# lefarov/Ape-X-DQN

Hardware: AMD Instinct MI355X
Metric: learner grad-steps/sec at batch 512, 84x84x4 dueling DQN (higher is better)
Workload: dtype fp32; 1 GPU; model=dueling NatureCNN (reference DuellingDQN, conv1=64), 4x84x84, A=4, global_batch=512, seq_len=1, parallelism=dp1, batch_scope=global, per_rank_rows=512, replay_per_gpu=100000, learner=fused/hip, hip_graphs=True

## Files before the change

### apex_dqn_amd/csrc/conv12_fused.hip

```cpp
#include "mfma_common.h"
#include "conv2_wfrag.h"
#include "cf_pack.h"

#define CF_THREADS 256
#define CF_PLANE 52224
#define CF_MAXIMG 64
#define CF_FRAME 7056
#define CF_NY2 12
#define CF_WAHEAD 3
#define CF_W3AHEAD 5
#define CF_W3EARLY 0

typedef float f32x16 __attribute__((ext_vector_type(16)));

struct Conv12Desc {
  const uint8_t* ring;
  const int32_t* slots;
  const float* w1;
  const float* w1b;
  const float* b1;
  const float* b1b;
  const bf16_t* w2;
  const bf16_t* w2_lo;
  const bf16_t* w2b;
// ... 3 lines not shown
  const float* b2;
  const float* b2b;
  bf16_t* y1;
  bf16_t* y1_lo;
  bf16_t* y2;
  bf16_t* y2_lo;
  uint4* w1frag;
  uint8_t* scratch;
  int N, C, img_switch, copy_n;
  float in_scale;
  uint64_t* probe;
  unsigned long long* wq;
  int bf16;
  int probe_split;
  const bf16_t* w3;
  const bf16_t* w3_lo;
  const bf16_t* w3b;
  const bf16_t* w3b_lo;
  const float* b3;
  const float* b3b;
  bf16_t* y3;
  bf16_t* y3_lo;
  uint4* w3frag;
};

template <int C>
__global__ void __launch_bounds__(256) cf_pack_kernel(CfPack p) {
  if ((int)blockIdx.x < p.nc2f) {
    c2f_pack_range(p.c2f, blockIdx.x * 256 + threadIdx.x, p.nc2f * 256);
    return;
  }
  if ((int)blockIdx.x < p.nc2f + p.nc3f) {
    c3f_pack_range(p.c3f, (blockIdx.x - p.nc2f) * 256 + threadIdx.x, p.nc3f * 256);
    return;
  }
  cf_pack_w1_block(p, C, (int)blockIdx.x - p.nc2f - p.nc3f, threadIdx.x);
}

__device__ __forceinline__ int cf_pix(int ih, int iw) { return ((ih & 1) * 2 + (iw & 1)) * 100 + (ih >> 1) * 10 + (iw >> 1); }
__device__ __forceinline__ int cf_off(int P, int c) { return (P << 7) + ((c ^ ((P >> 1) & 7)) << 4); }

__host__ __device__ constexpr int cf_young_stores(int ndw, bool split) {
  int n = 0;
  for (int q = ndw - 1; q < 12; ++q) n += (split || (q & 1) == 0) ? 1 : 0;
  return n;
}
// ... 85 lines not shown
      const float s0 = __shfl(ws, 4 * g, 64), s1 = __shfl(ws, 4 * g + 1, 64);
      const float s2 = __shfl(ws, 4 * g + 2, 64), s3 = __shfl(ws, 4 * g + 3, 64);
      bias1[nt] = (f32x4){bb.x - 1024.f * s0, bb.y - 1024.f * s1, bb.z - 1024.f * s2, bb.w - 1024.f * s3};
    }
    wf = d.wfrag + set * 2 * C2F_FRAGS + wv * 32 * 64 + lane;
    const float* B2 = set ? d.b2b : d.b2;
#pragma unroll
    for (int jh = 0; jh < 2; ++jh)
      bias2[jh] = *reinterpret_cast<const float4*>(B2 + nh * 32 + 8 * (2 * kp + jh) + 4 * kg);
    asm volatile("s_waitcnt vmcnt(0)" ::: "memory");
  };

  int q0[3];
#pragma unroll
  for (int mt = 0; mt < 3; ++mt) {
    const int r = mt * 32 + rr, oh = r / 10, ow = r - oh * 10;
    q0[mt] = (oh + kp) * 10 + ow;
  }

  const bool two = d.w1b != nullptr;
  int cur_set = -1;
  uint4 pend[3][2];
  int pend_img = -1;
  int yoff[3];
#pragma unroll
  for (int mt = 0; mt < 3; ++mt) {
    const int r = mt * 32 + rr, oh = r / 10, ow = r - oh * 10;
    yoff[mt] = (oh < 9 && ow < 9) ? ((oh * 9 + ow) * 64 + nh * 32 + 4 * kg) * 2 : -1;
  }
  auto store_y2 = [&](int q) {
    const int mt = q >> 2, jh = (q >> 1) & 1, plane = q & 1;
    const int jq = 2 * kp + jh;
    if (!SPLIT && plane) return;
    const uint8_t* base = reinterpret_cast<const uint8_t*>((plane ? d.y2_lo : d.y2) + (int64_t)pend_img * 5184);
    if (yoff[mt] >= 0) {
      const uint4 v = pend[mt][jh];
      *reinterpret_cast<uint2*>(const_cast<uint8_t*>(base) + (uint32_t)(yoff[mt] + 16 * jq)) =
          plane ? make_uint2(v.z, v.w) : make_uint2(v.x, v.y);
    }
  };
  bf16x8 wh3[CF_W3AHEAD + 1], wl3[CF_W3AHEAD + 1];
  auto w3row = [&](const int set3, const bool lo) -> const uint4* {
    return d.w3frag + (2 * set3 + (lo ? 1 : 0)) * C3F_FRAGS + (wv & 1) * 36 * 64 + lane;
  };
  auto wofs3 = [](int s) { return s * 64; };
  auto conv3_prefetch = [&](const int set3) {
// ... 108 lines not shown
            split_pk_bf16(v2, v3, h23, l23);
          } else {
            h01 = cvt_pk_bf16(v0, v1);
            h23 = cvt_pk_bf16(v2, v3);
          }
          if (oh < 7 && ow < 7) {
            const uint32_t off = (uint32_t)(((oh * 7 + ow) * 64 + c0) * 2);
            *reinterpret_cast<uint2*>(y3h + off) = make_uint2(h01, h23);
            if (SPLIT) *reinterpret_cast<uint2*>(y3l + off) = make_uint2(l01, l23);
          }
        }
      }
    }
    __syncthreads();
    if (it == 0) PROBE(d.probe, 4, PROBE_ITERS - 3, 3);
  };

  PROBE(d.probe, 4, PROBE_ITERS - 2, 0);
  if (cur < d.N) issue_dma(cur, 0);
  PROBE(d.probe, 4, PROBE_ITERS - 2, 1);
  for (int i = 0; cur < d.N; ++i) {
    const int img = cur;
    const bool more = nxt < d.N;
    const int set = (two && img >= d.img_switch) ? 1 : 0;
    if (set != cur_set) {
#ifdef APEX_PROBE
      if (i == 0 && (d.probe_split & 1)) asm volatile("s_waitcnt vmcnt(0)" ::: "memory");
      if (i == 0) PROBE(d.probe, 4, PROBE_ITERS - 2, 2);
#endif
      load_weights(set);
      cur_set = set;
      if (i == 0) PROBE(d.probe, 4, PROBE_ITERS - 2, 3);
      __syncthreads();
    }
    sl4_t nsl = (sl4_t){0, 0, 0, 0};
    if (more) nsl = image_slots(nxt);
    if (tid == 0) reinterpret_cast<volatile int*>(&q_img)[0] = more ? wq_next(d.wq, wq_seq, d.N) : d.N;
    PROBE(d.probe, 4, i, 0);
    const uint8_t* S = STG + (i & 1) * STGB;
    {
      auto load_tile = [&](int j, uint2* u) {
        int p = 16 * (th + 2 * j) + pl;
        if (j == 12) p = min(p, 399);
        const int oh = p / 20, ow = p - 20 * oh;
        const uint8_t* A = S + ((oh * 21 + ow) << 4);
#pragma unroll
// ... 43 lines not shown
          }
          if (pj >= 0) {
#pragma unroll
            for (int k = s2 * 8 / (2 * C); k < (s2 + 1) * 8 / (2 * C); ++k) epi_piece(k, pj, pacc, paccl);
          }
#pragma unroll
          for (int q = 0; q < (SPLIT ? 4 : 2); ++q) {
            __builtin_amdgcn_sched_group_barrier(0x008, 1, 0);
            __builtin_amdgcn_sched_group_barrier(0x002, SPLIT ? 3 : 5, 0);
          }
          __builtin_amdgcn_sched_barrier(0);
        }
      };
      uint2 u[2][2 * C];
      f32x4 a[2][2], al[2][2];
      load_tile(0, u[0]);
      load_tile(1, u[1]);
      __builtin_amdgcn_sched_barrier(0);
      mfma_tile(u[0], a[0], al[0], -1, nullptr, nullptr);
#pragma unroll
      for (int j = 1; j < 13; ++j) {
        if (j + 1 < 13) load_tile(j + 1, u[(j + 1) & 1]);
        if (j - 1 < NDW && more) issue_dma_piece(nsl, (i + 1) & 1, j - 1);
        if (i > 0) store_y2(j - 1);
        __builtin_amdgcn_sched_barrier(0);
        mfma_tile(u[j & 1], a[j & 1], al[j & 1], j - 1, a[(j - 1) & 1], al[(j - 1) & 1]);
      }
#pragma unroll
      for (int k = 0; k < 8; ++k) epi_piece(k, 12, a[0], al[0]);
    }
    PROBE(d.probe, 4, i, 1);
    static_assert(NDW <= 7, "the vmcnt below assumes the last DMA piece at tile <= 7");
    if (i > 0) asm volatile("s_waitcnt vmcnt(%0)" ::"n"(cf_young_stores(NDW, SPLIT)) : "memory");
    else asm volatile("s_waitcnt vmcnt(0)" ::: "memory");
    __syncthreads();
    const bool copy = img < d.copy_n;
    if (copy) {
      int tq = tid;
      asm volatile("" : "+v"(tq));
      const int cst = tq & 7;
      auto store_chunk = [&](const int r, const uint4 v) {
        const int k = tq + CF_THREADS * r;
        const int plane = k >= 3200 ? 1 : 0, kk = k - plane * 3200;
        const int P = kk >> 3, c = cst ^ ((P >> 1) & 7);
        const int cls = P / 100, q = P - cls * 100, a = q / 10, b = q - a * 10;
        const int ih = 2 * a + (cls >> 1), iw = 2 * b + (cls & 1);
        *reinterpret_cast<uint4*>((plane ? d.y1_lo : d.y1) + (int64_t)img * 25600 + (ih * 20 + iw) * 64 + c * 8) = v;
      };
      constexpr int NR = SPLIT ? 25 : 12, NB = SPLIT ? 5 : 4;
#pragma unroll
      for (int r0 = 0; r0 < NR; r0 += NB) {
        uint4 v[NB];
#pragma unroll
        for (int r = 0; r < NB; ++r)
          v[r] = *reinterpret_cast<const uint4*>(
              Y1 + (r0 + r) * 4096 + tq * 16 +
// ... 78 lines not shown
          const float v1 = fmaxf((bb.y + p0.y) + p1.y, 0.f);
          const float v2 = fmaxf((bb.z + p0.z) + p1.z, 0.f);
          const float v3 = fmaxf((bb.w + p0.w) + p1.w, 0.f);
          uint32_t h01, l01 = 0, h23, l23 = 0;
          if (SPLIT) {
            split_pk_bf16(v0, v1, h01, l01);
            split_pk_bf16(v2, v3, h23, l23);
          } else {
            h01 = cvt_pk_bf16(v0, v1);
            h23 = cvt_pk_bf16(v2, v3);
          }
          pend[mt][jh] = make_uint4(h01, h23, l01, l23);
        }
      }
    };
    if (kp == 0) finish(0, true);
    else finish(2, false);
    pend_img = img;
    __syncthreads();
    if (d.w3 != nullptr) conv3_image(img, set, STG + (i & 1) * STGB, i);
    cur = nxt;
    nxt = nn;
  }
  if (pend_img >= 0) {
#pragma unroll
    for (int q = 0; q < 12; ++q) store_y2(q);
  }
  PROBE(d.probe, 4, PROBE_ITERS - 1, 1);
#ifdef APEX_PROBE
  asm volatile("s_waitcnt vmcnt(0)" ::: "memory");
  if (d.probe != nullptr && blockIdx.x < PROBE_BLOCKS && (threadIdx.x & 63) == 0)
    d.probe[((blockIdx.x * 4 + (threadIdx.x >> 6)) * PROBE_ITERS + PROBE_ITERS - 1) * 4 + 3] =
        __builtin_amdgcn_s_memrealtime();
#endif
}

static int cf_launch_pack(const Conv12Desc& d, hipStream_t st) {
  const int sets = d.pack_sets & ((d.w1b != nullptr) ? 3 : 1);
  if (sets == 0) return 0;
  const bool s0 = sets & 1, s1 = (sets & 2) != 0;
  const bool c3 = d.w3 != nullptr && d.w3frag != nullptr;
  CfPack pk{C2fPack{{s0 ? d.w2 : nullptr, s0 ? d.w2_lo : nullptr, s1 ? d.w2b : nullptr, s1 ? d.w2b_lo : nullptr},
                    d.wfrag, 0},
            (s1 ? 4 : 2) * C2F_FRAGS / 256,
            C3fPack{{c3 && s0 ? d.w3 : nullptr, c3 && s0 ? d.w3_lo : nullptr, c3 && s1 ? d.w3b : nullptr,
                     c3 && s1 ? d.w3b_lo : nullptr}, d.w3frag},
            c3 ? (s1 ? 4 : 2) * C3F_FRAGS / 256 : 0,
// ... 20 lines not shown
APEX_EXPORT int apex_conv12_fused_fwd(Conv12Desc d, int grid, hipStream_t st) {
  if (d.N < 1) return 0;
  const bool sp = d.bf16 == 0;
  if (d.ring == nullptr || d.slots == nullptr || d.w1 == nullptr || d.b1 == nullptr || d.w2 == nullptr ||
      (sp && d.w2_lo == nullptr) || d.b2 == nullptr || d.y2 == nullptr || (sp && d.y2_lo == nullptr) ||
      d.wfrag == nullptr || d.scratch == nullptr || d.w1frag == nullptr)
    return (int)hipErrorInvalidValue;
  const bool two = d.w1b != nullptr;
  if (two && (d.b1b == nullptr || d.w2b == nullptr || (sp && d.w2b_lo == nullptr) || d.b2b == nullptr))
    return (int)hipErrorInvalidValue;
  if (d.copy_n > 0 && (d.y1 == nullptr || (sp && d.y1_lo == nullptr) || d.copy_n > d.N))
    return (int)hipErrorInvalidValue;
  if (d.w3 != nullptr &&
      (d.b3 == nullptr || d.y3 == nullptr || d.w3frag == nullptr || ((uintptr_t)d.w3frag & 15) || (sp && (d.w3_lo == nullptr || d.y3_lo == nullptr)) ||
       (two && (d.w3b == nullptr || d.b3b == nullptr || (sp && d.w3b_lo == nullptr))) ||
       (((uintptr_t)d.w3 | (uintptr_t)(sp ? d.w3_lo : d.w3) | (uintptr_t)(two ? d.w3b : d.w3) |
         (uintptr_t)(two && sp ? d.w3b_lo : d.w3) | (uintptr_t)d.b3 | (uintptr_t)(two ? d.b3b : d.b3)) & 15) ||
       (((uintptr_t)d.y3 | (uintptr_t)(sp ? d.y3_lo : d.y3)) & 7)))
    return (int)hipErrorInvalidValue;
  if ((((uintptr_t)d.w1 | (uintptr_t)(two ? d.w1b : d.w1) | (uintptr_t)d.b1 | (uintptr_t)(two ? d.b1b : d.b1) |
        (uintptr_t)d.w2 | (uintptr_t)d.w2_lo | (uintptr_t)d.b2 | (uintptr_t)d.y1 | (uintptr_t)d.y1_lo) & 15) ||
      (((uintptr_t)d.y2 | (uintptr_t)d.y2_lo | (uintptr_t)d.scratch) & 7) || ((uintptr_t)d.wfrag & 15))
    return (int)hipErrorInvalidValue;
  int G = grid > 0 ? grid : 256;
  if (G > d.N) G = d.N;
  if ((d.N + G - 1) / G > CF_MAXIMG) G = (d.N + CF_MAXIMG - 1) / CF_MAXIMG;
  const int err = cf_launch_pack(d, st);
  if (err) return err;
  switch (d.C * 2 + (sp ? 1 : 0)) {
    case 3: conv12_fused_kernel<1, true><<<G, CF_THREADS, 0, st>>>(d); break;
    case 5: conv12_fused_kernel<2, true><<<G, CF_THREADS, 0, st>>>(d); break;
    case 9: conv12_fused_kernel<4, true><<<G, CF_THREADS, 0, st>>>(d); break;
    case 2: conv12_fused_kernel<1, false><<<G, CF_THREADS, 0, st>>>(d); break;
    case 4: conv12_fused_kernel<2, false><<<G, CF_THREADS, 0, st>>>(d); break;
    case 8: conv12_fused_kernel<4, false><<<G, CF_THREADS, 0, st>>>(d); break;
    default: return (int)hipErrorInvalidValue;
  }
  APEX_CHECK_LAUNCH();
}
```

### apex_dqn_amd/learner/fused_learner.py

```python
from __future__ import annotations

from typing import Any, Dict, Optional

import torch

from ..config import ApexConfig
from ..models.dueling import DuellingDQN
from ..models.flat_params import (FlatLayout, flat_to_reference_state, nature_segments,
                                  reference_state_to_flat)
from ..ops.fused_ops import HipBackend, TorchBackend, split_into
from ..ops.switches import SW
from ..utils.checkpoint import (adopt_obs_scale, check_dist_head, check_noisy, layout_segments, load_checkpoint,
                                pack_flat_state, save_checkpoint, unpack_flat_state, checkpoint_network)
from .dp_step import DataParallelStep, Streams
from .is_norm import IsNormMixin
from .schedules import StepIndexMixin, target_ema_on


def _enable_sharding(replay, comm, rt, mcap: int = 0) -> None:
    if not replay.sharded:
        seed0 = comm.broadcast_int(int(rt.seed)) if hasattr(comm, "broadcast_int") else int(rt.seed)
        replay.enable_sharding(comm.rank, comm.world_size, shard_seed=(seed0 << 20) ^ 0x5EED,
                               group=comm.group, mcap=mcap)
    replay.shard_mcap = int(mcap)
# ... 303 lines not shown
        return kw if self.split else {}

    @property
    def _conv123(self) -> bool:
        return bool(self._c12) and 0 < 3 * self.B <= SW.conv123_max_images

    @property
    def _rows_first(self) -> int:
        return self.B if self.munchausen else 2 * self.B

    def forward_all(self, defer_head: bool = False) -> None:
        ops, rt, B = self.ops, self.rt, self.B
        Pb, P, Tb, T, Pl, Tl = self.Pb, self.P, self.Tb, self.T, self.Pl, self.Tl
        sp = self.split
        n, r1 = 3 * B, self._rows_first
        ring, slots = self._frame_src()
        if self._c12:
            c1, c2 = self._conv12_weights()
            online = 0 if self._frag_out is not None else 1
            c3 = self._conv3_weights() if self._conv123 else None
            ops.conv12_fwd(ring, slots, self.frames, rt.obs_scale, self.y1, self.y1_lo, self.y2,
                           self.y2_lo, c1, c2, rows_first=r1, copy_n=B,
                           pack_sets=online | (0 if self._tgt_current() else 2), c3=c3, y3=self.y3,
                           y3_lo=self.y3_lo)
        else:
            c2f = (Pb["w2"], None, Tb["w2"], None)
            ops.conv1_fwd_ring(ring, slots, self.frames, Pb["w1"], P["b1"], rt.obs_scale, self.y1,
                               Tb["w1"], T["b1"], r1, c2f=c2f)
            ops.conv_fwd(self.y1, Pb["w2"], P["b2"], 2, self.y2, Tb["w2"], T["b2"], r1)
        self._issue_params()
        if not self._conv123:
            ops.conv_fwd(self.y2, Pb["w3"], P["b3"], 1, self.y3, Tb["w3"], T["b3"], r1,
                         **self._lo(x_lo=self.y2_lo, w_lo=sp and Pl["w3"], w2_lo=sp and Tl["w3"], out_lo=self.y3_lo))
        self._wait_params()
        wfc, wfc_lo, bfc, wfc_t, wfc_t_lo, bfc_t = self._fc_weights()
        ops.fc_fwd(self.y3.reshape(n, 3136), wfc, bfc, self.h, wfc_t, bfc_t, r1,
                   c2d=(Pb["w2"], Pl["w2"] if sp else None), defer_head=defer_head,
                   **self._lo(x_lo=sp and self.y3_lo.reshape(n, 3136), w_lo=wfc_lo,
                              w2_lo=wfc_t_lo, out_lo=self.h_lo))

    def _conv12_weights(self):
        P, T, Pb, Tb, Pl, Tl = self.P, self.T, self.Pb, self.Tb, self.Pl, self.Tl
        sp = self.split
        return ((P["w1"], P["b1"], T["w1"], T["b1"]),
                (Pb["w2"], Pl["w2"] if sp else None, P["b2"], Tb["w2"], Tl["w2"] if sp else None, T["b2"]))

    def _conv3_weights(self):
# ... 606 lines not shown
```

### apex_dqn_amd/ops/conv.py

```python
from __future__ import annotations

from typing import Dict, Optional, Tuple


import torch

from . import _lib
from .switches import SW


class Workspace:
    def __init__(self):
        self.bufs: Dict[Tuple, torch.Tensor] = {}

    def get(self, key, numel: int, device, dtype=torch.float32) -> torch.Tensor:
        k = (key, numel, str(device), dtype)
        t = self.bufs.get(k)
        if t is None:
            t = torch.empty(numel, dtype=dtype, device=device)
            self.bufs[k] = t
        return t

    work_queue = False

# ... 201 lines not shown


def conv12_frag_out(ws: "Workspace", w1: torch.Tensor, w1_off: int, w2_off: int, scale: float,
                    w3_off: Optional[int] = None, target: bool = False):
    C = int(w1.shape[1])
    dev = w1.device
    fo = _lib.CfFragOut()
    s = 1 if target else 0
    fo.w1frag = ws.get(("cf_w1frag",), CF_W1FRAG_BYTES, dev, torch.uint8).data_ptr() + s * 1024 * C * 16
    fo.c2f = ws.get(("cf_c2f_wfrag",), 4 * 8192 * 16, dev, torch.uint8).data_ptr() + s * 2 * 8192 * 16
    fo.w1_off, fo.w2_off, fo.C, fo.in_scale = int(w1_off), int(w2_off), C, float(scale)
    if w3_off is not None:
        fo.c3f = ws.get(("cf_c3f",), C3F_BYTES, dev, torch.uint8).data_ptr() + s * 2 * 4608 * 16
        fo.w3_off = int(w3_off)
    return fo


def conv12_fused_fwd(lib, ws: "Workspace", ring: torch.Tensor, slots: torch.Tensor, w1: torch.Tensor,
                     b1: torch.Tensor, w2: torch.Tensor, w2_lo: torch.Tensor, b2: torch.Tensor, scale: float,
                     y2: torch.Tensor, y2_lo: torch.Tensor, y1: Optional[torch.Tensor] = None,
                     y1_lo: Optional[torch.Tensor] = None, copy_n: int = 0, w1b=None, b1b=None, w2b=None,
                     w2b_lo=None, b2b=None, rows_first: int = 0, grid: int = 0,
                     probe: Optional[torch.Tensor] = None, pack_sets: int = 3, probe_split: int = 0,
                     c3=None, y3: Optional[torch.Tensor] = None, y3_lo: Optional[torch.Tensor] = None) -> None:
    N, C = slots.shape
    sp = w2_lo is not None
    assert slots.dtype == torch.int32 and slots.is_contiguous() and int(w1.shape[1]) == C
    assert tuple(y2.shape[:4]) == (N, 9, 9, 64) and y2.is_contiguous() and y2.dtype == torch.bfloat16
    assert not sp or (y2_lo is not None and tuple(y2_lo.shape) == (N, 9, 9, 64))
    d = _conv12_desc(ws, ring, slots, w1, b1, w2, w2_lo, b2, scale, w1b, b1b, w2b, w2b_lo, b2b, c3)
    d.img_switch = int(rows_first) if w1b is not None else N
    if copy_n > 0:
        assert y1 is not None and (y1_lo is not None or not sp) and y1.shape[0] >= copy_n and \
            tuple(y1.shape[1:]) == (20, 20, 64) and y1.is_contiguous()
        d.y1, d.y1_lo = y1.data_ptr(), (y1_lo.data_ptr() if sp else 0)
    d.copy_n = int(copy_n)
    d.y2, d.y2_lo = y2.data_ptr(), (y2_lo.data_ptr() if sp else 0)
    d.pack_sets = int(pack_sets)
    d.N = N
    d.probe = _lib.ptr(probe)
    d.probe_split = int(probe_split)
    d.wq = ws.wq(("cf_wq", N, int(grid)), ring.device, overlapped=False)
    if c3 is not None:
        assert y3 is not None and tuple(y3.shape[:4]) == (N, 7, 7, 64) and y3.is_contiguous()
        assert not sp or (y3_lo is not None and tuple(y3_lo.shape[:4]) == (N, 7, 7, 64))
        d.y3, d.y3_lo = y3.data_ptr(), (y3_lo.data_ptr() if sp else 0)
    _lib.check(lib.apex_conv12_fused_fwd(d, int(grid), _lib.stream_ptr()), "conv12_fused_fwd")


def conv_fwd(lib, x: torch.Tensor, w: torch.Tensor, b: torch.Tensor, stride: int, out: torch.Tensor,
             w2=None, b2=None, rows_first: int = 0, x_lo=None, w_lo=None, w2_lo=None, out_lo=None,
             packed: bool = False) -> None:
    N, H, W, Cin = x.shape
    Cout, KH, KW, _ = w.shape
    OH, OW = out.shape[1], out.shape[2]
    if SW.conv2_img and (H, W, Cin, Cout, KH, KW, stride) == (20, 20, 64, 64, 4, 4, 2) and \
            hasattr(lib, "apex_conv2_img_fwd"):
        conv2_img_fwd(lib, x, w, b, out, w2, b2, rows_first, x_lo=x_lo, w_lo=w_lo, w2_lo=w2_lo, out_lo=out_lo,
                      packed=packed)
        return
    d = _conv_desc(x=x.data_ptr(), w=w.data_ptr(), bias=b.data_ptr(), y=out.data_ptr(), N=N, H=H, W=W,
                   Cin=Cin, OH=OH, OW=OW, Cout=Cout, KH=KH, KW=KW, stride=stride, mode=1, relu=1,
# ... 172 lines not shown

def _splits(Mred: int, target_rows: int, max_rows: int) -> Tuple[int, int]:
    rows = max(_WG_ROWS, min(max_rows, (target_rows // _WG_ROWS) * _WG_ROWS))
    return (Mred + rows - 1) // rows, rows


def conv2_wgrad_rows_covers(x_shape, dy_shape, KH: int, stride: int, split: bool, rows: int) -> bool:
    return (bool(split) and KH == 4 and stride == 2 and len(x_shape) == 4 and len(dy_shape) == 4
            and tuple(x_shape[1:]) == (20, 20, 64) and tuple(dy_shape[1:]) == (9, 9, 64)
            and x_shape[0] == dy_shape[0] and x_shape[0] > 0
            and rows > 0 and rows % _WG_ROWS == 0 and rows <= _WG_TBL)


def conv2_wgrad_rows_pick(x_shape, dy_shape, KH: int, stride: int, split: bool, rows: int,
                          force: Optional[bool] = None) -> bool:
    covers = conv2_wgrad_rows_covers(x_shape, dy_shape, KH, stride, split, rows)
    if force is not None:
        if force and not covers:
            raise ValueError("conv2_wgrad_rows does not cover this problem")
        return bool(force)
    return covers and bool(SW.conv2_wgrad_rows) and x_shape[0] >= SW.conv2_wgrad_rows_min


def conv_wgrad(lib, ws: Workspace, dy: torch.Tensor, x: torch.Tensor, KH: int, stride: int,
               dw_out: torch.Tensor, db_out: torch.Tensor, target_rows: int = 0, jobs: Optional[list] = None,
               dy_lo=None, x_lo=None, rows_kernel: Optional[bool] = None) -> None:
    N, OH, OW, Co = dy.shape
    if target_rows <= 0:
        small = N < 256
        target_rows = {3: SW.wg_rows3, 4: SW.wg_rows2}.get(KH) or \
            ((192 if small else 384) if KH == 3 else (352 if small else 704))
    _, H, W, Cin = x.shape
    Kc = KH * KH * Cin
    Mred = N * OH * OW
    nsplit, rows = _splits(Mred, target_rows, _WG_TBL)
    slab = ws.get(("wg", Co, Kc), nsplit * Co * Kc, dy.device)
    bslab = ws.get(("wgb", Co, Kc), nsplit * Co, dy.device)
    d = _wg_desc(dy=dy.data_ptr(), x=x.data_ptr(), slab=slab.data_ptr(), bias_slab=bslab.data_ptr(), N=N,
                 H=H, W=W, Cin=Cin, OH=OH, OW=OW, KH=KH, KW=KH, stride=stride, mode=1, Co=Co, Kc=Kc, ldd=Co,
                 rows_per_split=rows, Mred=Mred, dy_lo=_lib.ptr(dy_lo), x_lo=_lib.ptr(x_lo))
    launch, what = lib.apex_conv_wgrad, "conv_wgrad"
    if conv2_wgrad_rows_pick(x.shape, dy.shape, KH, stride, dy_lo is not None and x_lo is not None, rows,
                             rows_kernel):
        launch, what = lib.apex_conv2_wgrad_rows, "conv2_wgrad_rows"
    if jobs is not None:
        _lib.check(launch(d, None, None, nsplit, 1.0, _lib.stream_ptr()), what)
        jobs.append(dict(slab=slab, bslab=bslab, out=dw_out, bout=db_out, n=Co * Kc, nsplit=nsplit, nb=Co,
                         s2dC=0, Kc=Kc, scale=1.0))
        return
    _lib.check(launch(d, dw_out.data_ptr(), db_out.data_ptr(), nsplit, 1.0, _lib.stream_ptr()), what)
# ... 208 lines not shown
```

### apex_dqn_amd/ops/conv_sigs.py

```python
from __future__ import annotations

import ctypes

c_p = ctypes.c_void_p
c_i = ctypes.c_int
c_i64 = ctypes.c_int64
c_f = ctypes.c_float


class Conv2ImgDesc(ctypes.Structure):
    _fields_ = [("x", c_p), ("w", c_p), ("w2", c_p), ("bias", c_p), ("bias2", c_p), ("y", c_p),
                ("N", c_i), ("img_switch", c_i), ("x_lo", c_p), ("w_lo", c_p), ("w2_lo", c_p), ("y_lo", c_p),
                ("wfrag", c_p), ("wfrag_ready", c_i)]


class Conv12Desc(ctypes.Structure):
    _fields_ = [("ring", c_p), ("slots", c_p), ("w1", c_p), ("w1b", c_p), ("b1", c_p), ("b1b", c_p),
                ("w2", c_p), ("w2_lo", c_p), ("w2b", c_p), ("w2b_lo", c_p), ("wfrag", c_p), ("pack_sets", c_i),
                ("b2", c_p), ("b2b", c_p), ("y1", c_p), ("y1_lo", c_p), ("y2", c_p), ("y2_lo", c_p),
                ("w1frag", c_p), ("scratch", c_p), ("N", c_i), ("C", c_i), ("img_switch", c_i), ("copy_n", c_i),
                ("in_scale", ctypes.c_float), ("probe", c_p), ("wq", c_p), ("bf16", c_i), ("probe_split", c_i),
                ("w3", c_p), ("w3_lo", c_p), ("w3b", c_p), ("w3b_lo", c_p), ("b3", c_p), ("b3b", c_p),
                ("y3", c_p), ("y3_lo", c_p), ("w3frag", c_p)]


class Conv2DgradImgDesc(ctypes.Structure):
    _fields_ = [("dy", c_p), ("w", c_p), ("mask", c_p), ("dx", c_p), ("N", c_i), ("dy_lo", c_p), ("w_lo", c_p),
                ("dx_lo", c_p), ("wfrag", c_p), ("wfrag_ready", c_i), ("wq", c_p), ("cls_split", c_i)]


class Conv21BwdDesc(ctypes.Structure):
    _fields_ = [("dy", c_p), ("dy_lo", c_p), ("w", c_p), ("w_lo", c_p), ("mask", c_p), ("wfrag", c_p),
                ("wfrag_ready", c_i), ("ring", c_p), ("slots", c_p), ("zero16", c_p), ("slab", c_p),
                ("bias_slab", c_p), ("dx", c_p), ("dx_lo", c_p), ("wq", c_p), ("N", c_i), ("C", c_i)]


class C2dPackJob(ctypes.Structure):
    _fields_ = [("w", c_p), ("w_lo", c_p), ("out", c_p)]


class Conv3DgradImgDesc(ctypes.Structure):
    _fields_ = [("dy", c_p), ("w", c_p), ("mask", c_p), ("dx", c_p), ("N", c_i)]


class Conv3DgradSplitDesc(ctypes.Structure):
    _fields_ = [("dy", c_p), ("dy_lo", c_p), ("w", c_p), ("w_lo", c_p), ("mask", c_p), ("dx", c_p),
                ("dx_lo", c_p), ("N", c_i), ("H", c_i), ("W", c_i), ("Cout", c_i), ("Cin", c_i), ("KH", c_i),
                ("KW", c_i), ("stride", c_i)]


def declare(lib: ctypes.CDLL) -> None:
    from ._lib import ConvDesc, WgradDesc
    sigs = {
        "apex_conv2_img_fwd": ([Conv2ImgDesc, c_i, c_p], c_i),
        "apex_conv12_fused_fwd": ([Conv12Desc, c_i, c_p], c_i),
        "apex_conv12_pack": ([Conv12Desc, c_p], c_i),
        "apex_conv2_dgrad_img": ([Conv2DgradImgDesc, c_i, c_p], c_i),
        "apex_conv3_dgrad_img": ([Conv3DgradImgDesc, c_i, c_p], c_i),
        "apex_conv3_dgrad_img_split": ([Conv3DgradSplitDesc, c_i, c_p], c_i),
        "apex_conv21_bwd_fused": ([Conv21BwdDesc, c_i, c_p], c_i),
        "apex_conv_fwd": ([ConvDesc, c_p], c_i),
        "apex_fc_gemm128": ([ConvDesc, c_p, c_i64, c_i, c_i, c_i, C2dPackJob, c_p], c_i),
        "apex_conv_wgrad": ([WgradDesc, c_p, c_p, c_i, c_f, c_p], c_i),
        "apex_conv2_wgrad_rows": ([WgradDesc, c_p, c_p, c_i, c_f, c_p], c_i),
        "apex_pack_dgrad_weights": ([c_p, c_p, c_p, c_p, c_p, c_p, c_p], c_i),
    }
    for name, (args, res) in sigs.items():
        fn = getattr(lib, name, None)
        if fn is None:
            continue
        fn.argtypes = args
        fn.restype = res
```

### apex_dqn_amd/ops/fused_ops.py

```python
from __future__ import annotations

import ctypes
from typing import Dict, Optional

import numpy as np
import torch

from . import _lib
from . import conv as C
from . import reference as R
from ..learner.rescale import rescale_target
from .switches import SW


def join(hi: torch.Tensor, lo: Optional[torch.Tensor], dtype=torch.float32) -> torch.Tensor:
    return hi.to(dtype) if lo is None else hi.to(dtype) + lo.to(dtype)


def _head_dtype(t: torch.Tensor):
    return torch.float64 if t.dtype == torch.float64 else torch.float32


def split_into(v: torch.Tensor, hi: torch.Tensor, lo: Optional[torch.Tensor]) -> None:
    hi.copy_(v.reshape(hi.shape))
# ... 19 lines not shown
        dt = torch.float32 if out_lo is not None else self.dtype
        split_into(R.conv1_fwd(frames, w, b, scale, dt), out, out_lo)

    def conv1_fwd_ring(self, ring, slots, frames_buf, w, b, scale, out, w2=None, b2=None, rows_first=0, w32=None,
                       w2_32=None, out_lo=None, c2f=None):
        from ..replay.gpu_replay import from_s2d
        frames = frames_buf[:slots.shape[0]]
        n, c = slots.shape
        frames.copy_(from_s2d(ring[slots.long()].reshape(n * c, 84, 84)).reshape(n, c, 84, 84))
        wa, wb = (w32, w2_32) if out_lo is not None else (w, w2)
        if w2 is None:
            self.conv1_fwd(frames, wa, b, scale, out, out_lo)
        else:
            r = rows_first
            self.conv1_fwd(frames[:r], wa, b, scale, out[:r], None if out_lo is None else out_lo[:r])
            self.conv1_fwd(frames[r:], wb, b2, scale, out[r:], None if out_lo is None else out_lo[r:])

    def conv12_pack(self, c1, c2, scale, sets=2, c3=None):
        """Repack the fused conv12 kernel's weight fragments of ``sets`` (bit 0 online, bit
        1 target; HIP backend only) -- after the target weights change; ``c3``: the fused
        conv3's too."""

    def conv12_fwd(self, ring, slots, frames_buf, scale, y1, y1_lo, y2, y2_lo, c1, c2, rows_first=0, copy_n=None,
                   pack_sets=3, c3=None, y3=None, y3_lo=None):
        w1, b1, w1b, b1b = c1
        w2, w2l, b2, w2b, w2bl, b2b = c2
        self.conv1_fwd_ring(ring, slots, frames_buf, w1.to(y1.dtype), b1, scale, y1,
                            None if w1b is None else w1b.to(y1.dtype), b1b, rows_first, w32=w1, w2_32=w1b,
                            out_lo=y1_lo)
        self.conv_fwd(y1, w2, b2, 2, y2, w2b, b2b, rows_first, x_lo=y1_lo, w_lo=w2l, w2_lo=w2bl, out_lo=y2_lo)
        if c3 is not None:
            w3, w3l, b3, w3b, w3bl, b3b = c3
            self.conv_fwd(y2, w3, b3, 1, y3, w3b, b3b, rows_first, x_lo=y2_lo, w_lo=w3l, w2_lo=w3bl, out_lo=y3_lo)

    def conv_fwd(self, x, w, b, stride, out, w2=None, b2=None, rows_first=0, x_lo=None, w_lo=None, w2_lo=None,
                 out_lo=None):
        dt = torch.float32 if x_lo is not None else self.dtype
        xf = join(x, x_lo) if x_lo is not None else x
        if w2 is None:
            split_into(R.conv_fwd(xf, join(w, w_lo), b, stride, dt), out, out_lo)
        else:
            r = rows_first
            split_into(R.conv_fwd(xf[:r], join(w, w_lo), b, stride, dt), out[:r], None if out_lo is None else out_lo[:r])
            split_into(R.conv_fwd(xf[r:], join(w2, w2_lo), b2, stride, dt), out[r:],
                       None if out_lo is None else out_lo[r:])

    def fc_fwd(self, x, w, b, out, w2=None, b2=None, rows_first=0, x_lo=None, w_lo=None, w2_lo=None, out_lo=None,
# ... 612 lines not shown
    def conv1_fwd_ring(self, ring, slots, frames_buf, w, b, scale, out, w2=None, b2=None, rows_first=0, w32=None,
                       w2_32=None, out_lo=None, c2f=None):
        if not self.native_conv:
            return super().conv1_fwd_ring(ring, slots, frames_buf, w, b, scale, out, w2, b2, rows_first, w32, w2_32,
                                          out_lo)
        c2f = c2f if (c2f is not None and SW.c2f_pack) else None
        C.conv1_s2d_fwd(self.lib, self.ws, ring, slots, w, b, scale, out, w2, b2, rows_first, w32=w32, w2_32=w2_32,
                        out_lo=out_lo, c2f=c2f)
        if c2f is not None:
            self._c2f_packed = tuple(_lib.ptr(t) for t in c2f)

    def _conv12_native(self) -> bool:
        return self.native_conv and SW.conv12_fused and hasattr(self.lib, "apex_conv12_fused_fwd")

    def conv12_pack(self, c1, c2, scale, sets=2, c3=None):
        if not self._conv12_native():
            return
        w1, b1, w1b, b1b = c1
        w2, w2l, b2, w2b, w2bl, b2b = c2
        C.conv12_pack(self.lib, self.ws, w1, b1, w2, w2l, b2, scale, w1b=w1b, b1b=b1b, w2b=w2b, w2b_lo=w2bl,
                      b2b=b2b, sets=sets, c3=c3)

    def conv12_fwd(self, ring, slots, frames_buf, scale, y1, y1_lo, y2, y2_lo, c1, c2, rows_first=0, copy_n=None,
                   pack_sets=3, c3=None, y3=None, y3_lo=None):
        if not self._conv12_native():
            return super().conv12_fwd(ring, slots, frames_buf, scale, y1, y1_lo, y2, y2_lo, c1, c2, rows_first,
                                      copy_n, c3=c3, y3=y3, y3_lo=y3_lo)
        w1, b1, w1b, b1b = c1
        w2, w2l, b2, w2b, w2bl, b2b = c2
        n = slots.shape[0] if copy_n is None else int(copy_n)
        C.conv12_fused_fwd(self.lib, self.ws, ring, slots, w1, b1, w2, w2l, b2, scale, y2, y2_lo, y1=y1, y1_lo=y1_lo,
                           copy_n=n, w1b=w1b, b1b=b1b, w2b=w2b, w2b_lo=w2bl, b2b=b2b, rows_first=rows_first,
                           pack_sets=pack_sets, c3=c3, y3=y3, y3_lo=y3_lo)

    def conv_fwd(self, x, w, b, stride, out, w2=None, b2=None, rows_first=0, x_lo=None, w_lo=None, w2_lo=None,
                 out_lo=None):
        if not self.native_conv:
            return super().conv_fwd(x, w, b, stride, out, w2, b2, rows_first, x_lo, w_lo, w2_lo, out_lo)
        key = (_lib.ptr(w), _lib.ptr(w_lo), _lib.ptr(w2), _lib.ptr(w2_lo))
        packed = stride == 2 and getattr(self, "_c2f_packed", None) == key
        if packed:
            self._c2f_packed = None
        C.conv_fwd(self.lib, x, w, b, stride, out, w2, b2, rows_first, x_lo=x_lo, w_lo=w_lo, w2_lo=w2_lo,
                   out_lo=out_lo, packed=packed)

    def fc_fwd(self, x, w, b, out, w2=None, b2=None, rows_first=0, x_lo=None, w_lo=None, w2_lo=None, out_lo=None,
               c2d=None, defer_head=False, ksplit=0):
        if not self.native_conv:
            return super().fc_fwd(x, w, b, out, w2, b2, rows_first, x_lo, w_lo, w2_lo, out_lo)
        M, K = x.shape[0], x[0].numel()
        if w.shape[0] % 128 == 0 and K % 64 == 0 and hasattr(self.lib, "apex_fc_gemm128"):
            defer = defer_head and w2 is not None and b is not None and b2 is not None and \
                2 * (M // 3) == rows_first and M % 3 == 0
            tiles = C.row_tiles_host(M, rows_first if w2 is not None else None, 128) * (w.shape[0] // 128)
            if ksplit > 0:
                ks = int(ksplit)
# ... 491 lines not shown
```

### apex_dqn_amd/ops/switches.py

```python
from __future__ import annotations

import dataclasses
import os
from dataclasses import dataclass
from typing import Any, Dict


@dataclass
class Switches:
    conv2_img: bool = True
    c2f_pack: bool = True
    conv12_fused: bool = True
    conv123_max_images: int = 1 << 20
    conv12_bf16: bool = True
    conv3_dgrad_img: bool = True
    conv2_dgrad_img: bool = True
    conv3_dgrad_img_split: bool = True
    conv3_dgrad_img_split_min: int = 74
    conv2_dgrad_cls_max: int = 256
    conv21_bwd_fused: bool = True
    opt_frags: bool = True
    fc_epi_in_head: bool = True
    bwd_branches: bool = True
    actor_fc_ksplit: int = 4
    fc_wgrad_main: str = "auto"
    fc_ksplit_max: int = 0
    work_queue: str = "auto"
    wg_rows3: int = 0
    wg_rows2: int = 0
    conv2_wgrad_rows: bool = True
    conv2_wgrad_rows_min: int = 512
    impala_wg_target: int = 512
    impala_slab_cap: int = 8 << 20
    resblock_r16: int = 14
    impala_pool_wgrad: bool = True
    isplit_bands: str = ""
    dp_fc_shard_branch: bool = False
    dp_branch_one_wait: bool = True
    dp_fc_split_rows: int = -1
    dp_norm_split: bool = True

    @classmethod
    def from_env(cls, spec: str = None) -> "Switches":
        sw = cls()
        spec = os.environ.get("APEX_SWITCHES", "") if spec is None else spec
        for item in spec.split(","):
            item = item.strip()
            if not item:
                continue
            if "=" not in item:
                raise ValueError(f"APEX_SWITCHES item must be name=value, got {item!r}")
            k, v = item.split("=", 1)
            f = {f.name: f for f in dataclasses.fields(cls)}.get(k)
            if f is None:
# ... 21 lines not shown
```

Baseline: 2946 grad-steps/s (batch 512).

## Skip y2 stores for target-net images and add per-image conv3 wgrad kernel

The fused conv1/2/3 forward kernel now writes y2 only for the first y2_n images (the online batch) when conv3 is fused. Target-network images never need y2 for backward, so this removes their global stores and the vmcnt wait on them. Separately, it adds a per-image double-buffered split-bf16 MFMA conv3 weight-gradient kernel with slab reduction. That kernel is gated behind a switch that defaults to off.

```diff
diff --git a/apex_dqn_amd/csrc/conv12_fused.hip b/apex_dqn_amd/csrc/conv12_fused.hip
--- a/apex_dqn_amd/csrc/conv12_fused.hip
+++ b/apex_dqn_amd/csrc/conv12_fused.hip
@@ -49,6 +49,7 @@
   bf16_t* y3;
   bf16_t* y3_lo;
   uint4* w3frag;
+  int y2_n;
 };
 
 template <int C>
@@ -180,6 +181,7 @@
   int cur_set = -1;
   uint4 pend[3][2];
   int pend_img = -1;
+  const int y2_lim = d.y2_n;
   int yoff[3];
 #pragma unroll
   for (int mt = 0; mt < 3; ++mt) {
@@ -334,6 +336,7 @@
   for (int i = 0; cur < d.N; ++i) {
     const int img = cur;
     const bool more = nxt < d.N;
+    const bool st_prev = pend_img >= 0 && pend_img < y2_lim;
     const int set = (two && img >= d.img_switch) ? 1 : 0;
     if (set != cur_set) {
 #ifdef APEX_PROBE
@@ -423,7 +426,7 @@
       for (int j = 1; j < 13; ++j) {
         if (j + 1 < 13) load_tile(j + 1, u[(j + 1) & 1]);
         if (j - 1 < NDW && more) issue_dma_piece(nsl, (i + 1) & 1, j - 1);
-        if (i > 0) store_y2(j - 1);
+        if (st_prev) store_y2(j - 1);
         __builtin_amdgcn_sched_barrier(0);
         mfma_tile(u[j & 1], a[j & 1], al[j & 1], j - 1, a[(j - 1) & 1], al[(j - 1) & 1]);
       }
@@ -432,7 +435,7 @@
     }
     PROBE(d.probe, 4, i, 1);
     static_assert(NDW <= 7, "the vmcnt below assumes the last DMA piece at tile <= 7");
-    if (i > 0) asm volatile("s_waitcnt vmcnt(%0)" ::"n"(cf_young_stores(NDW, SPLIT)) : "memory");
+    if (st_prev) asm volatile("s_waitcnt vmcnt(%0)" ::"n"(cf_young_stores(NDW, SPLIT)) : "memory");
     else asm volatile("s_waitcnt vmcnt(0)" ::: "memory");
     __syncthreads();
     const bool copy = img < d.copy_n;
@@ -557,7 +560,7 @@
     cur = nxt;
     nxt = nn;
   }
-  if (pend_img >= 0) {
+  if (pend_img >= 0 && pend_img < y2_lim) {
 #pragma unroll
     for (int q = 0; q < 12; ++q) store_y2(q);
   }
@@ -624,6 +627,7 @@
         (uintptr_t)d.w2 | (uintptr_t)d.w2_lo | (uintptr_t)d.b2 | (uintptr_t)d.y1 | (uintptr_t)d.y1_lo) & 15) ||
       (((uintptr_t)d.y2 | (uintptr_t)d.y2_lo | (uintptr_t)d.scratch) & 7) || ((uintptr_t)d.wfrag & 15))
     return (int)hipErrorInvalidValue;
+  if (d.w3 == nullptr || d.y2_n <= 0 || d.y2_n > d.N) d.y2_n = d.N;
   int G = grid > 0 ? grid : 256;
   if (G > d.N) G = d.N;
   if ((d.N + G - 1) / G > CF_MAXIMG) G = (d.N + CF_MAXIMG - 1) / CF_MAXIMG;
diff --git a/apex_dqn_amd/csrc/conv3_wgrad_img.hip b/apex_dqn_amd/csrc/conv3_wgrad_img.hip
--- /dev/null
+++ b/apex_dqn_amd/csrc/conv3_wgrad_img.hip
@@ -0,0 +1,162 @@
+#include "igemm_wgrad.h"
+
+#define C3W_THREADS 512
+#define C3W_DY 8192
+#define C3W_XROWS 88
+#define C3W_X (C3W_XROWS * 128)
+#define C3W_BUF (2 * C3W_DY + 2 * C3W_X)
+#define C3W_NPIECE (2 * 8 + 2 * 11)
+#define C3W_PPW ((C3W_NPIECE + 7) / 8)
+static_assert(2 * C3W_BUF <= 160 * 1024, "LDS");
+
+__device__ __forceinline__ bf16x8 c3w_frag(const uint8_t* img, int row0, int col0, int lane) {
+  const int g = lane >> 4, q = (lane >> 2) & 3, pcol = lane & 3;
+  const int rA = row0 + 8 * g + q;
+  const int cbyte = (col0 + 4 * pcol) * 2;
+  const int c16 = cbyte >> 4, within = cbyte & 15;
+  const lds_s16x4* pa = (const lds_s16x4*)(img + swz_tr(rA, c16) + within);
+  const lds_s16x4* pb = (const lds_s16x4*)(img + swz_tr(rA + 4, c16) + within);
+  s16x4 lo = __builtin_amdgcn_ds_read_tr16_b64_v4i16(const_cast<lds_s16x4*>(pa));
+  s16x4 hi = __builtin_amdgcn_ds_read_tr16_b64_v4i16(const_cast<lds_s16x4*>(pb));
+  typedef short s16x8 __attribute__((ext_vector_type(8)));
+  s16x8 v = (s16x8){lo[0], lo[1], lo[2], lo[3], hi[0], hi[1], hi[2], hi[3]};
+  return __builtin_bit_cast(bf16x8, v);
+}
+
+__global__ void __launch_bounds__(C3W_THREADS, 1) conv3_wgrad_img_kernel(WgradDesc d) {
+  __shared__ __attribute__((aligned(16))) uint8_t smem[2 * C3W_BUF];
+  const int tid = threadIdx.x, lane = tid & 63;
+  const int wv = __builtin_amdgcn_readfirstlane(tid >> 6);
+  const int ch = wv & 1, kq = wv >> 1;
+  const int b = (int)blockIdx.x, G = (int)gridDim.x;
+  const int i0 = (int)(((int64_t)b * d.N) / G), i1 = (int)(((int64_t)(b + 1) * d.N) / G);
+
+  for (int i = tid; i < 2 * C3W_BUF / 16; i += C3W_THREADS)
+    *reinterpret_cast<uint4*>(smem + i * 16) = make_uint4(0, 0, 0, 0);
+
+  uint32_t voff[C3W_PPW];
+#pragma unroll
+  for (int k = 0; k < C3W_PPW; ++k) {
+    const int p = wv + 8 * k;
+    const bool isx = p >= 16;
+    const int lp = isx ? (p - 16) % 11 : (p & 7);
+    const int R = lp * 8 + (lane >> 3);
+    const int s = ((R >> 1) & 1) | (((R >> 3) & 1) << 1);
+    const int c = (lane & 7) ^ (s << 1);
+    const int oh = R / 9, ow = R - 9 * oh;
+    const bool ok = isx ? R < 81 : (oh < 7 && ow < 7);
+    const int pix = isx ? R : oh * 7 + ow;
+    voff[k] = ok && p < C3W_NPIECE ? (uint32_t)(pix * 128 + c * 16) : 0xffffffffu;
+  }
+  const uint32_t lds0 = (uint32_t)(uintptr_t)(__attribute__((address_space(3))) uint8_t*)smem;
+  auto issue_dma = [&](int img, int buf) {
+#pragma unroll
+    for (int k = 0; k < C3W_PPW; ++k) {
+      const int p = wv + 8 * k;
+      if (p < C3W_NPIECE) {
+        const bool isx = p >= 16;
+        const bool lo = isx ? p >= 27 : p >= 8;
+        const int lp = isx ? (p - 16) % 11 : (p & 7);
+        const uint8_t* src = isx ? reinterpret_cast<const uint8_t*>(lo ? d.x_lo : d.x) + (int64_t)img * (81 * 128)
+                                 : reinterpret_cast<const uint8_t*>(lo ? d.dy_lo : d.dy) + (int64_t)img * (49 * 128);
+        const uint32_t dst = __builtin_amdgcn_readfirstlane(
+            lds0 + (uint32_t)(buf * C3W_BUF + (isx ? 2 * C3W_DY + (lo ? C3W_X : 0) : (lo ? C3W_DY : 0)) + lp * 1024));
+        if (voff[k] != 0xffffffffu) dma16_s(src, voff[k], dst);
+      }
+    }
+  };
+
+  f32x4 acc[2][9], accb[2], accb_sum[2];
+#pragma unroll
+  for (int i = 0; i < 2; ++i) {
+    accb[i] = (f32x4){0.f, 0.f, 0.f, 0.f};
+    accb_sum[i] = (f32x4){0.f, 0.f, 0.f, 0.f};
+#pragma unroll
+    for (int j = 0; j < 9; ++j) acc[i][j] = (f32x4){0.f, 0.f, 0.f, 0.f};
+  }
+  const bf16x8 ones = __builtin_bit_cast(bf16x8, make_uint4(0x3f803f80u, 0x3f803f80u, 0x3f803f80u, 0x3f803f80u));
+  const bool do_bias = d.bias_slab != nullptr && kq == 0;
+
+  __syncthreads();
+  if (i0 < i1) issue_dma(i0, 0);
+  for (int img = i0, buf = 0; img < i1; ++img, buf ^= 1) {
+    asm volatile("s_waitcnt vmcnt(0)" ::: "memory");
+    __syncthreads();
+    if (img + 1 < i1) issue_dma(img + 1, buf ^ 1);
+    const uint8_t* DH = smem + buf * C3W_BUF;
+    const uint8_t* DL = DH + C3W_DY;
+    const uint8_t* XH = DH + 2 * C3W_DY;
+    const uint8_t* XL = XH + C3W_X;
+#pragma unroll
+    for (int kk = 0; kk < 2; ++kk) {
+      bf16x8 a[2], al[2];
+#pragma unroll
+      for (int i = 0; i < 2; ++i) {
+        a[i] = c3w_frag(DH, 32 * kk, 32 * ch + 16 * i, lane);
+        al[i] = c3w_frag(DL, 32 * kk, 32 * ch + 16 * i, lane);
+      }
+#pragma unroll
+      for (int j = 0; j < 9; ++j) {
+        const int col0 = 144 * kq + 16 * j, tap = col0 >> 6, ci0 = col0 & 63;
+        const int kh = tap / 3, toff = 9 * kh + (tap - 3 * kh);
+        const bf16x8 x = c3w_frag(XH, 32 * kk + toff, ci0, lane);
+        const bf16x8 xl = c3w_frag(XL, 32 * kk + toff, ci0, lane);
+#pragma unroll
+        for (int i = 0; i < 2; ++i) {
+          acc[i][j] = __builtin_amdgcn_mfma_f32_16x16x32_bf16(x, al[i], acc[i][j], 0, 0, 0);
+          acc[i][j] = __builtin_amdgcn_mfma_f32_16x16x32_bf16(xl, a[i], acc[i][j], 0, 0, 0);
+          acc[i][j] = __builtin_amdgcn_mfma_f32_16x16x32_bf16(x, a[i], acc[i][j], 0, 0, 0);
+        }
+      }
+      if (do_bias) {
+#pragma unroll
+        for (int i = 0; i < 2; ++i) {
+          accb[i] = __builtin_amdgcn_mfma_f32_16x16x32_bf16(ones, al[i], accb[i], 0, 0, 0);
+          accb[i] = __builtin_amdgcn_mfma_f32_16x16x32_bf16(ones, a[i], accb[i], 0, 0, 0);
+        }
+      }
+    }
+    if (do_bias && (((img - i0) & 3) == 3 || img + 1 == i1)) {
+#pragma unroll
+      for (int i = 0; i < 2; ++i) {
+        accb_sum[i] += accb[i];
+        accb[i] = (f32x4){0.f, 0.f, 0.f, 0.f};
+      }
+    }
+  }
+
+  const int g = lane >> 4, pl = lane & 15;
+  float* slab = d.slab + (int64_t)b * 64 * 576;
+#pragma unroll
+  for (int i = 0; i < 2; ++i)
+#pragma unroll
+    for (int j = 0; j < 9; ++j)
+      *reinterpret_cast<f32x4*>(slab + (32 * ch + 16 * i + pl) * 576 + 144 * kq + 16 * j + 4 * g) = acc[i][j];
+  if (do_bias && g == 0) {
+#pragma unroll
+    for (int i = 0; i < 2; ++i) d.bias_slab[(int64_t)b * 64 + 32 * ch + 16 * i + pl] = accb_sum[i][0];
+  }
+}
+
+static bool conv3_wgrad_img_covers(const WgradDesc& d) {
+  return d.mode == 1 && d.H == 9 && d.W == 9 && d.Cin == 64 && d.OH == 7 && d.OW == 7 && d.KH == 3 && d.KW == 3 &&
+         d.stride == 1 && d.pad_h == 0 && d.pad_w == 0 && d.Co == 64 && d.Kc == 576 && d.ldd == 64 &&
+         d.dy != nullptr && d.x != nullptr && d.dy_lo != nullptr && d.x_lo != nullptr && d.slab != nullptr &&
+         d.norm_part == nullptr && d.N > 0 && d.Mred == d.N * 49 &&
+         ((((uintptr_t)d.dy | (uintptr_t)d.x | (uintptr_t)d.dy_lo | (uintptr_t)d.x_lo | (uintptr_t)d.slab) & 15) == 0);
+}
+
+APEX_EXPORT int apex_slab_reduce(const float* slab, int nsplit, int64_t n, float scale, float* out, const float* bslab,
+                                 int nb, float* bout, int s2dC, int Kc, hipStream_t st);
+
+APEX_EXPORT int apex_conv3_wgrad_img(WgradDesc d, float* out, float* bout, int nsplit, float scale, hipStream_t st) {
+  if (!conv3_wgrad_img_covers(d)) return (int)hipErrorInvalidValue;
+  if (nsplit < 1 || nsplit > d.N) return (int)hipErrorInvalidValue;
+  conv3_wgrad_img_kernel<<<nsplit, C3W_THREADS, 0, st>>>(d);
+  hipError_t e = hipGetLastError();
+  if (e != hipSuccess) return (int)e;
+  if (out != nullptr)
+    return apex_slab_reduce(d.slab, nsplit, (int64_t)64 * 576, scale, out, d.bias_slab, d.bias_slab ? 64 : 0, bout, 0,
+                            576, st);
+  return 0;
+}
diff --git a/apex_dqn_amd/learner/fused_learner.py b/apex_dqn_amd/learner/fused_learner.py
--- a/apex_dqn_amd/learner/fused_learner.py
+++ b/apex_dqn_amd/learner/fused_learner.py
@@ -349,7 +349,7 @@
             ops.conv12_fwd(ring, slots, self.frames, rt.obs_scale, self.y1, self.y1_lo, self.y2,
                            self.y2_lo, c1, c2, rows_first=r1, copy_n=B,
                            pack_sets=online | (0 if self._tgt_current() else 2), c3=c3, y3=self.y3,
-                           y3_lo=self.y3_lo)
+                           y3_lo=self.y3_lo, y2_n=B if (c3 is not None and SW.conv12_y2_rows) else None)
         else:
             c2f = (Pb["w2"], None, Tb["w2"], None)
             ops.conv1_fwd_ring(ring, slots, self.frames, Pb["w1"], P["b1"], rt.obs_scale, self.y1,
diff --git a/apex_dqn_amd/ops/conv.py b/apex_dqn_amd/ops/conv.py
--- a/apex_dqn_amd/ops/conv.py
+++ b/apex_dqn_amd/ops/conv.py
@@ -247,7 +247,8 @@
                      y1_lo: Optional[torch.Tensor] = None, copy_n: int = 0, w1b=None, b1b=None, w2b=None,
                      w2b_lo=None, b2b=None, rows_first: int = 0, grid: int = 0,
                      probe: Optional[torch.Tensor] = None, pack_sets: int = 3, probe_split: int = 0,
-                     c3=None, y3: Optional[torch.Tensor] = None, y3_lo: Optional[torch.Tensor] = None) -> None:
+                     c3=None, y3: Optional[torch.Tensor] = None, y3_lo: Optional[torch.Tensor] = None,
+                     y2_n: Optional[int] = None) -> None:
     N, C = slots.shape
     sp = w2_lo is not None
     assert slots.dtype == torch.int32 and slots.is_contiguous() and int(w1.shape[1]) == C
@@ -263,6 +264,9 @@
     d.y2, d.y2_lo = y2.data_ptr(), (y2_lo.data_ptr() if sp else 0)
     d.pack_sets = int(pack_sets)
     d.N = N
+    if y2_n is not None:
+        assert 1 <= int(y2_n) <= N
+        d.y2_n = int(y2_n)
     d.probe = _lib.ptr(probe)
     d.probe_split = int(probe_split)
     d.wq = ws.wq(("cf_wq", N, int(grid)), ring.device, overlapped=False)
@@ -481,10 +485,49 @@
     return covers and bool(SW.conv2_wgrad_rows) and x_shape[0] >= SW.conv2_wgrad_rows_min
 
 
+def conv3_wgrad_img_covers(x_shape, dy_shape, KH: int, stride: int, split: bool) -> bool:
+    return (bool(split) and KH == 3 and stride == 1 and len(x_shape) == 4 and len(dy_shape) == 4
+            and tuple(x_shape[1:]) == (9, 9, 64) and tuple(dy_shape[1:]) == (7, 7, 64)
+            and x_shape[0] == dy_shape[0] and x_shape[0] > 0)
+
+
+def conv3_wgrad_img_pick(x_shape, dy_shape, KH: int, stride: int, split: bool, force: Optional[bool] = None) -> bool:
+    covers = conv3_wgrad_img_covers(x_shape, dy_shape, KH, stride, split)
+    if force is not None:
+        if force and not covers:
+            raise ValueError("conv3_wgrad_img does not cover this problem")
+        return bool(force)
+    return covers and bool(SW.conv3_wgrad_img) and x_shape[0] >= SW.conv3_wgrad_img_min
+
+
+def _conv3_wgrad_img(lib, ws: Workspace, dy, x, dw_out, db_out, jobs, dy_lo, x_lo, grid: int) -> None:
+    N = dy.shape[0]
+    for t in (dy, x, dy_lo, x_lo):
+        assert t.is_contiguous() and t.dtype == torch.bfloat16
+    assert dy_lo.shape == dy.shape and x_lo.shape == x.shape
+    G = max(1, min(N, int(grid) if grid > 0 else int(SW.conv3_wgrad_img_grid)))
+    slab = ws.get(("wg3img", G), G * 64 * 576, dy.device)
+    bslab = ws.get(("wg3imgb", G), G * 64, dy.device)
+    d = _wg_desc(dy=dy.data_ptr(), x=x.data_ptr(), slab=slab.data_ptr(), bias_slab=bslab.data_ptr(), N=N, H=9, W=9,
+                 Cin=64, OH=7, OW=7, KH=3, KW=3, stride=1, mode=1, Co=64, Kc=576, ldd=64, rows_per_split=0,
+                 Mred=N * 49, dy_lo=dy_lo.data_ptr(), x_lo=x_lo.data_ptr())
+    if jobs is not None:
+        _lib.check(lib.apex_conv3_wgrad_img(d, None, None, G, 1.0, _lib.stream_ptr()), "conv3_wgrad_img")
+        jobs.append(dict(slab=slab, bslab=bslab, out=dw_out, bout=db_out, n=64 * 576, nsplit=G, nb=64, s2dC=0,
+                         Kc=576, scale=1.0))
+        return
+    _lib.check(lib.apex_conv3_wgrad_img(d, dw_out.data_ptr(), db_out.data_ptr(), G, 1.0, _lib.stream_ptr()),
+               "conv3_wgrad_img")
+
+
 def conv_wgrad(lib, ws: Workspace, dy: torch.Tensor, x: torch.Tensor, KH: int, stride: int,
                dw_out: torch.Tensor, db_out: torch.Tensor, target_rows: int = 0, jobs: Optional[list] = None,
-               dy_lo=None, x_lo=None, rows_kernel: Optional[bool] = None) -> None:
+               dy_lo=None, x_lo=None, rows_kernel: Optional[bool] = None, img_kernel: Optional[bool] = None,
+               img_grid: int = 0) -> None:
     N, OH, OW, Co = dy.shape
+    if conv3_wgrad_img_pick(x.shape, dy.shape, KH, stride, dy_lo is not None and x_lo is not None, img_kernel):
+        _conv3_wgrad_img(lib, ws, dy, x, dw_out, db_out, jobs, dy_lo, x_lo, img_grid)
+        return
     if target_rows <= 0:
         small = N < 256
         target_rows = {3: SW.wg_rows3, 4: SW.wg_rows2}.get(KH) or \
diff --git a/apex_dqn_amd/ops/conv_sigs.py b/apex_dqn_amd/ops/conv_sigs.py
--- a/apex_dqn_amd/ops/conv_sigs.py
+++ b/apex_dqn_amd/ops/conv_sigs.py
@@ -21,7 +21,7 @@
                 ("w1frag", c_p), ("scratch", c_p), ("N", c_i), ("C", c_i), ("img_switch", c_i), ("copy_n", c_i),
                 ("in_scale", ctypes.c_float), ("probe", c_p), ("wq", c_p), ("bf16", c_i), ("probe_split", c_i),
                 ("w3", c_p), ("w3_lo", c_p), ("w3b", c_p), ("w3b_lo", c_p), ("b3", c_p), ("b3b", c_p),
-                ("y3", c_p), ("y3_lo", c_p), ("w3frag", c_p)]
+                ("y3", c_p), ("y3_lo", c_p), ("w3frag", c_p), ("y2_n", c_i)]
 
 
 class Conv2DgradImgDesc(ctypes.Structure):
@@ -63,6 +63,7 @@
         "apex_fc_gemm128": ([ConvDesc, c_p, c_i64, c_i, c_i, c_i, C2dPackJob, c_p], c_i),
         "apex_conv_wgrad": ([WgradDesc, c_p, c_p, c_i, c_f, c_p], c_i),
         "apex_conv2_wgrad_rows": ([WgradDesc, c_p, c_p, c_i, c_f, c_p], c_i),
+        "apex_conv3_wgrad_img": ([WgradDesc, c_p, c_p, c_i, c_f, c_p], c_i),
         "apex_pack_dgrad_weights": ([c_p, c_p, c_p, c_p, c_p, c_p, c_p], c_i),
     }
     for name, (args, res) in sigs.items():
diff --git a/apex_dqn_amd/ops/fused_ops.py b/apex_dqn_amd/ops/fused_ops.py
--- a/apex_dqn_amd/ops/fused_ops.py
+++ b/apex_dqn_amd/ops/fused_ops.py
@@ -65,7 +65,7 @@
         conv3's too."""
 
     def conv12_fwd(self, ring, slots, frames_buf, scale, y1, y1_lo, y2, y2_lo, c1, c2, rows_first=0, copy_n=None,
-                   pack_sets=3, c3=None, y3=None, y3_lo=None):
+                   pack_sets=3, c3=None, y3=None, y3_lo=None, y2_n=None):
         w1, b1, w1b, b1b = c1
         w2, w2l, b2, w2b, w2bl, b2b = c2
         self.conv1_fwd_ring(ring, slots, frames_buf, w1.to(y1.dtype), b1, scale, y1,
@@ -724,7 +724,7 @@
                       b2b=b2b, sets=sets, c3=c3)
 
     def conv12_fwd(self, ring, slots, frames_buf, scale, y1, y1_lo, y2, y2_lo, c1, c2, rows_first=0, copy_n=None,
-                   pack_sets=3, c3=None, y3=None, y3_lo=None):
+                   pack_sets=3, c3=None, y3=None, y3_lo=None, y2_n=None):
         if not self._conv12_native():
             return super().conv12_fwd(ring, slots, frames_buf, scale, y1, y1_lo, y2, y2_lo, c1, c2, rows_first,
                                       copy_n, c3=c3, y3=y3, y3_lo=y3_lo)
@@ -733,7 +733,7 @@
         n = slots.shape[0] if copy_n is None else int(copy_n)
         C.conv12_fused_fwd(self.lib, self.ws, ring, slots, w1, b1, w2, w2l, b2, scale, y2, y2_lo, y1=y1, y1_lo=y1_lo,
                            copy_n=n, w1b=w1b, b1b=b1b, w2b=w2b, w2b_lo=w2bl, b2b=b2b, rows_first=rows_first,
-                           pack_sets=pack_sets, c3=c3, y3=y3, y3_lo=y3_lo)
+                           pack_sets=pack_sets, c3=c3, y3=y3, y3_lo=y3_lo, y2_n=y2_n)
 
     def conv_fwd(self, x, w, b, stride, out, w2=None, b2=None, rows_first=0, x_lo=None, w_lo=None, w2_lo=None,
                  out_lo=None):
diff --git a/apex_dqn_amd/ops/switches.py b/apex_dqn_amd/ops/switches.py
--- a/apex_dqn_amd/ops/switches.py
+++ b/apex_dqn_amd/ops/switches.py
@@ -12,6 +12,7 @@
     c2f_pack: bool = True
     conv12_fused: bool = True
     conv123_max_images: int = 1 << 20
+    conv12_y2_rows: bool = True
     conv12_bf16: bool = True
     conv3_dgrad_img: bool = True
     conv2_dgrad_img: bool = True
@@ -30,6 +31,9 @@
     wg_rows2: int = 0
     conv2_wgrad_rows: bool = True
     conv2_wgrad_rows_min: int = 512
+    conv3_wgrad_img: bool = False
+    conv3_wgrad_img_min: int = 512
+    conv3_wgrad_img_grid: int = 128
     impala_wg_target: int = 512
     impala_slab_cap: int = 8 << 20
     resblock_r16: int = 14
```

Result: no change. 2981 grad-steps/s (batch 512) (median of 6 runs) (+1.2%).
